# jai1215snu/ShiftedScaleQuantization

Hardware: AMD Instinct MI355X
Metric: Gelem/s shifted-scale q/dq + recon iters/s, ResNet-18 W2A4; top-1 vs ref (higher is better)
Workload: dtype f32; 1 GPU; resnet18 W2A4 bias_cal+bias_ch_quant, 1024 calib samples: A4 per-tensor q/dq of act [1024,64,56,56] + W2 per-channel q/dq of all 21 conv/fc weights (8-bit stem/head); parallelism=dp1

## Files before the change

shiftedscalequantization_amd/csrc/conv_wgrad.hip:

```cpp
#include <stdlib.h>

#include <algorithm>
#include <type_traits>

#include "ssq_common.h"

namespace ssq {

typedef float f32x16 __attribute__((ext_vector_type(16)));

constexpr int kUnr = 2;

struct WgradGeo {
  int Nb, C, H, W, Co, OH, OW, R, S, st, pad, G, Cig, Cog;
  int Ncol;
  int WM;
  int Pq;
  int lda;
  int chunks_per_n;
  int nchunks;
  int cps;
  int nsplit;
  int in_rows;
  int ci_span;
// ... 574 lines not shown
        const int rr = (int)fdiv((uint32_t)rem, dWp), cc = rem - rr * Wp;
        const int ih = rr - pad, iw = cc - pad;
        v[u] = 0.0f;
        if (e < tot && ih >= 0 && ih < H && iw >= 0 && iw < W) v[u] = xb[(int64_t)j * C * HW + ih * W + iw];
      }
#pragma unroll
      for (int u = 0; u < U; ++u)
        if (e0 + 256 * u < tot) xs[e0 + 256 * u] = v[u];
    }
    __syncthreads();
    for (int p0 = tid; p0 < totp; p0 += 256 * kPf) {
      float g[kPf];
#pragma unroll
      for (int k = 0; k < kPf; ++k) {
        const int p = p0 + 256 * k;
        const int j = (int)fdiv((uint32_t)p, dOHW);
        g[k] = 0.0f;
        if (p < totp) g[k] = db[(int64_t)j * C * OHW + (p - j * OHW)];
      }
#pragma unroll 1
      for (int k = 0; k < kPf; ++k) {
        const int p = p0 + 256 * k;
        if (p >= totp) break;
        const int j = (int)fdiv((uint32_t)p, dOHW), q = p - j * OHW;
        const int oh = (int)fdiv((uint32_t)q, dOW), ow = q - oh * OW;
        const float* xr = xs + j * HpWp + oh * st * Wp + ow * st;
#pragma unroll
        for (int kk = 0; kk < RSMAX; ++kk) {
          if (kk < RS) {
            const int r = kk / S, q2 = kk - r * S;
            acc[kk] = __fadd_rn(acc[kk], __fmul_rn(g[0], xr[r * Wp + q2]));
          }
        }
#pragma unroll
        for (int t = 0; t + 1 < kPf; ++t) g[t] = g[t + 1];
      }
    }
  }
#pragma unroll
  for (int j = 0; j < RSMAX; ++j) {
    float v = acc[j];
#pragma unroll
    for (int o = 32; o >= 1; o >>= 1) v = __fadd_rn(v, __shfl_xor(v, o));
    if (lane == 0) red[w][j] = v;
  }
  __syncthreads();
  if (tid < RS)
    part[((int64_t)split * C + c) * RS + tid] =
        __fadd_rn(__fadd_rn(__fadd_rn(red[0][tid], red[1][tid]), red[2][tid]), red[3][tid]);
}

static bool is_depthwise(int64_t C, int64_t Co, int64_t G) { return G == C && G == Co && G > 1; }
static int dw_stage(int64_t H, int64_t W, int64_t pad, int spl) {
  const int64_t b = (H + 2 * pad) * (W + 2 * pad) * (int64_t)sizeof(float);
  if (b > 4096) return 0;
  return (int)std::max<int64_t>(1, std::min<int64_t>(spl, 32 * 1024 / b));
}
static int dw_band_rows(int64_t H, int64_t W, int64_t R, int64_t st, int64_t pad, int64_t OH) {
  const int64_t Wp = W + 2 * pad, row = Wp * (int64_t)sizeof(float);
  if ((H + 2 * pad) * row <= 8192) return (int)OH;
  const int64_t rows = std::max<int64_t>(R, 8192 / row);
  return (int)std::min<int64_t>(OH, (rows - R) / st + 1);
}
static bool dw_lds_ok(int64_t H, int64_t W, int64_t pad) {
  return (H + 2 * pad) * (W + 2 * pad) * (int64_t)sizeof(float) <= 128 * 1024;
}

static int dw_splits(int64_t Nb, int64_t C, int* spl) {
  int64_t ns = std::max<int64_t>(1, std::min<int64_t>(Nb, (1024 + C - 1) / C));
  *spl = (int)((Nb + ns - 1) / ns);
  while (Nb % *spl) ++*spl;
  return (int)(Nb / *spl);
}

static size_t wgrad_lds(int wm, int pq, int64_t xtile) {
  return sizeof(float) * (2 * (size_t)(64 * wm) * (pq + 1) + 2 * (size_t)(xtile + 1));
}

static int wgrad_plan(int64_t Nb, int64_t C, int64_t H, int64_t W, int64_t Co, int64_t R,
                      int64_t S, int64_t st, int64_t pad, int64_t G, WgradGeo& g,
                      size_t* lds_bytes) {
  SSQ_REQUIRE(Nb >= 1 && C >= 1 && H >= 1 && W >= 1 && Co >= 1 && R >= 1 && S >= 1 && st >= 1 &&
                  pad >= 0 && G >= 1 && C % G == 0 && Co % G == 0,
              SSQ_E_ARG, "ssq_conv_wgrad: bad geometry");
  const int64_t OH = (H + 2 * pad - R) / st + 1, OW = (W + 2 * pad - S) / st + 1;
  SSQ_REQUIRE(OH >= 1 && OW >= 1 && Nb * C * H * W < (1ll << 31) && Nb * Co * OH * OW < (1ll << 31),
              SSQ_E_ARG, "ssq_conv_wgrad: sizes");
  g.Nb = (int)Nb; g.C = (int)C; g.H = (int)H; g.W = (int)W; g.Co = (int)Co;
  g.OH = (int)OH; g.OW = (int)OW; g.R = (int)R; g.S = (int)S; g.st = (int)st; g.pad = (int)pad;
  g.G = (int)G; g.Cig = (int)(C / G); g.Cog = (int)(Co / G);
  g.Ncol = g.Cig * g.R * g.S;
  const int RS = g.R * g.S;
  const int64_t Wp = W + 2 * pad;
  static const int64_t max_lds = [] {
    const char* v = getenv("SSQ_K17_MAXLDS");
    return (int64_t)(v && *v ? atoll(v) : 160 * 1024);
  }();
  double best = 1e300;
  for (int wm : {1, 2, 4}) {
    for (int pq : {128, 64}) {
      const int TM = 64 * wm, TN = 256 / wm;
      const int64_t span = std::min<int64_t>(g.Cig, (TN - 1) / RS + 2);
      const int64_t orows = (pq - 1 + OW - 1) / OW + 1;
      const int64_t in_rows = (orows - 1) * st + R;
      const int64_t xtile = span * in_rows * Wp;
      if ((int64_t)wgrad_lds(wm, pq, xtile) > max_lds) continue;
      const int64_t cpn = (OH * OW + pq - 1) / pq;
      const int64_t tiles = ((g.Cog + TM - 1) / TM) * ((g.Ncol + TN - 1) / TN);
      const double dma = (double)(std::min<int64_t>(TM, g.Cog) * ((pq + 63) / 64) +
                                  span * in_rows * ((W + 63) / 64)) / 4.0;
      const double cost = (double)tiles * Nb * (2.0 * OH * OW + cpn * (40.0 + dma));
      if (cost < best) {
        best = cost;
        g.WM = wm;
        g.Pq = pq;
        g.ci_span = (int)span;
        g.in_rows = (int)in_rows;
        g.xtile = (int)xtile;
      }
    }
  }
  SSQ_REQUIRE(best < 1e300, SSQ_E_ARG, "ssq_conv_wgrad: input rows too wide for the LDS tile");
  const int TM = 64 * g.WM, TN = 256 / g.WM;
  g.lda = g.Pq + 1;
  g.chunks_per_n = (int)((OH * OW + g.Pq - 1) / g.Pq);
  g.nchunks = g.Nb * g.chunks_per_n;
  g.m_tiles = (g.Cog + TM - 1) / TM;
  g.n_tiles = (g.Ncol + TN - 1) / TN;
  const int64_t tiles = (int64_t)g.n_tiles * g.m_tiles * g.G;
  int nsplit = (int)std::max<int64_t>(1, std::min<int64_t>(g.nchunks / 2, (512 + tiles - 1) / tiles));
  g.cps = (g.nchunks + nsplit - 1) / nsplit;
  g.nsplit = (g.nchunks + g.cps - 1) / g.cps;
  *lds_bytes = wgrad_lds(g.WM, g.Pq, g.xtile);
  return SSQ_OK;
}

constexpr int kBandMaxNI = 20;
__device__ float g_band_zero_page[4 * 64];

struct BandGeo {
  int C, H, W, Co, OW, OHW, Cig, Cog;
  int RB, Q, Qp, PA, IR, PXrow, PXci;
  int TMc, CBc;
  int bufsz;
  int d16;
  int ni_w;
  int bands_per_n, nchunks, cps, nsplit, m_tiles, n_tiles, remap;
  FastDiv dPA, dPXci, dPXrow;
};

template <int N>
using IntC = std::integral_constant<int, N>;

template <int WMX, int ST, int V, int NWV>
__global__ __launch_bounds__(64 * NWV, 1) void wgrad_band_stage1(const float* __restrict__ x,
                                                                 const float* __restrict__ dy,
                                                                 BandGeo g, float* __restrict__ part) {
  static_assert(NWV == 4 || NWV == 8, "4 or 8 waves");
  constexpr int WNX = 4 / WMX;
  constexpr int kSlots = kBandMaxNI * 4 / NWV;
  extern __shared__ float lds[];
  const int tid = threadIdx.x, lane = tid & 63;
  const int wave = __builtin_amdgcn_readfirstlane(tid >> 6);
  const int wt = wave & 3, role = wave >> 2;
  const int wm = wt / WNX, wn = wt - wm * WNX;
  int wg = blockIdx.x;
  const int tiles = g.m_tiles * g.n_tiles;
  if (g.remap) {
    const int per = (int)gridDim.x >> 3;
    wg = (wg & 7) * per + (wg >> 3);
  }
  const int split = wg / tiles, tile = wg - split * tiles;
  const int mt = tile / g.n_tiles, nt = tile - mt * g.n_tiles;
  const int co0 = mt * g.TMc, ci0 = nt * g.CBc;
  const int c_begin = split * g.cps, c_end = min(c_begin + g.cps, g.nchunks);
  const int abytes = g.TMc * g.PA;
  const int n16 = g.d16 ? min(kSlots, (g.bufsz / 256 - wave + NWV - 1) / NWV) : 0;
  const int n4 = g.d16 ? 0 : (g.bufsz / 64 - wave + NWV - 1) / NWV;

  int soff[kSlots], meta[kSlots];
#pragma unroll
  for (int i = 0; i < kSlots; ++i) {
    soff[i] = 0;
    meta[i] = 0;
    if (i < n16) {
      const int o = (wave + NWV * i) * 256 + lane * 4;
      if (o < abytes) {
        const int row = (int)fdiv((uint32_t)o, g.dPA), col = o - row * g.PA;
        if (col < g.Q && co0 + row < g.Cog) {
          soff[i] = (co0 + row) * g.OHW + col;
          meta[i] = 1;
        }
      } else {
        const int o2 = o - abytes;
        const int cl = (int)fdiv((uint32_t)o2, g.dPXci), rem = o2 - cl * g.PXci;
        const int ir = (int)fdiv((uint32_t)rem, g.dPXrow), iw = rem - ir * g.PXrow - 4;
        if (cl < g.CBc && ci0 + cl < g.Cig && ir < g.IR && iw >= 0 && iw < g.W) {
          soff[i] = ((ci0 + cl) * g.H + ir) * g.W + iw;
          meta[i] = 2 | (ir << 2);
        }
      }
    }
  }
  struct Band {
    const float* ab;
    const float* xb;
    int ih0;
  };
  auto band_of = [&](int c) {
    const int n = c / g.bands_per_n;
    const int oh0 = (c - n * g.bands_per_n) * g.RB;
    const int ih0 = oh0 * ST - 1;
    return Band{dy + (int64_t)n * g.Co * g.OHW + oh0 * g.OW,
                x + (int64_t)n * g.C * g.H * g.W + (int64_t)ih0 * g.W, ih0};
  };
  auto stage16 = [&](const Band& bd, int b) {
    const float* zero = g_band_zero_page + lane * 4;
    float* dst = lds + b * g.bufsz + wave * 256;
#pragma unroll
    for (int i = 0; i < kSlots; ++i) {
      if (i < n16) {
        const int kind = meta[i] & 3;
        const unsigned ih = (unsigned)(bd.ih0 + (meta[i] >> 2));
        const bool ok = (kind == 1) | ((kind == 2) & (ih < (unsigned)g.H));
        const uint64_t pa = (uint64_t)(bd.ab + soff[i]), px = (uint64_t)(bd.xb + soff[i]);
        const uint64_t p = ok ? (kind == 1 ? pa : px) : (uint64_t)zero;
        __builtin_amdgcn_global_load_lds((const void*)p, (void*)(dst + i * NWV * 256), 16, 0, 0);
      }
    }
  };
  const int HW = g.H * g.W;
  auto stage4 = [&](const Band& bd, int b, int i0, int i1) {
    const float* zero = g_band_zero_page + lane;
    float* dst = lds + b * g.bufsz + wave * 64;
    for (int i = i0; i < i1; ++i) {
      const int o = (wave + NWV * i) * 64 + lane;
      const float* src = zero;
      if ((wave + NWV * i) * 64 < abytes) {
        const int row = (int)fdiv((uint32_t)o, g.dPA), col = o - row * g.PA;
        if (col < g.Q && co0 + row < g.Cog) src = bd.ab + (co0 + row) * g.OHW + col;
      } else {
        const int o2 = o - abytes;
        const int cl = (int)fdiv((uint32_t)o2, g.dPXci), rem = o2 - cl * g.PXci;
        const int ir = (int)fdiv((uint32_t)rem, g.dPXrow), iw = rem - ir * g.PXrow - 4;
        const unsigned ih = (unsigned)(bd.ih0 + ir);
        if (cl < g.CBc && ci0 + cl < g.Cig && ir < g.IR && iw >= 0 && iw < g.W &&
            ih < (unsigned)g.H)
          src = bd.xb + (ci0 + cl) * HW + ir * g.W + iw;
      }
      __builtin_amdgcn_global_load_lds((const void*)src, (void*)(dst + i * NWV * 64), 4, 0, 0);
    }
  };

  typedef float f32x4v __attribute__((ext_vector_type(4)));
  typedef float f32x2v __attribute__((ext_vector_type(2)));
  const int h = lane >> 5, l32 = lane & 31;
  const int arow = (wm * 32 + l32) * g.PA;
  const int xrow = abytes + (wn * 32 + l32) * g.PXci;
  const int q0 = h * (g.Qp >> 1);
  const int ngroups = g.Qp / (2 * V);
  const int last_row = (g.Q - 1) / g.OW, last_col = (g.Q - 1) - last_row * g.OW;
  constexpr int NW = (V - 1) * ST + 3;
  const int per_step = (n4 + max(1, ngroups / 2) - 1) / max(1, ngroups / 2);
  if (c_begin < c_end) {
    const Band bd = band_of(c_begin);
    if (g.d16) stage16(bd, 0);
    else stage4(bd, 0, 0, n4);
  }

  auto body = [&](auto t0c, auto t1c) {
    constexpr int T0 = decltype(t0c)::value, T1 = decltype(t1c)::value, NT = T1 - T0;
    constexpr int R0 = T0 / 3, NR = (T1 - 1) / 3 - R0 + 1;
    f32x16 acc[NT];
#pragma unroll
    for (int t = 0; t < NT; ++t) acc[t] = f32x16{0};
    auto fetch = [&](const float* L, int q, int orow, int ow, float (&a)[V],
                     float (&w)[NR][NW]) {
      if constexpr (V == 4) {
        const f32x4v av = *(const f32x4v*)(L + arow + q);
        a[0] = av.x; a[1] = av.y; a[2] = av.z; a[3] = av.w;
      } else if constexpr (V == 2) {
        const f32x2v av = *(const f32x2v*)(L + arow + q);
        a[0] = av.x; a[1] = av.y;
      } else {
        a[0] = L[arow + q];
      }
      int xr_row = orow, xr_col = ow;
      if (q >= g.Q) {
        xr_row = last_row;
        xr_col = last_col - (V - 1);
      }
      const float* xr0 = L + xrow + (xr_row * ST + R0) * g.PXrow + xr_col * ST + 3;
#pragma unroll
      for (int r = 0; r < NR; ++r) {
        const float* xr = xr0 + r * g.PXrow;
        if constexpr (V == 4) {
          w[r][0] = xr[0];
          const f32x4v t1 = *(const f32x4v*)(xr + 1);
          w[r][1] = t1.x; w[r][2] = t1.y; w[r][3] = t1.z; w[r][4] = t1.w;
          if constexpr (ST == 1) {
            w[r][5] = xr[5];
          } else {
            const f32x4v t2 = *(const f32x4v*)(xr + 5);
            w[r][5] = t2.x; w[r][6] = t2.y; w[r][7] = t2.z; w[r][8] = t2.w;
          }
        } else {
#pragma unroll
          for (int j = 0; j < NW; ++j) w[r][j] = xr[j];
        }
      }
    };
    auto mfmas = [&](const float (&a)[V], const float (&w)[NR][NW]) {
#pragma unroll
      for (int r = 0; r < NR; ++r)
#pragma unroll
        for (int v = 0; v < V; ++v)
#pragma unroll
          for (int s = 0; s < 3; ++s) {
            const int tap = (R0 + r) * 3 + s;
            if (tap >= T0 && tap < T1)
              acc[tap - T0] = __builtin_amdgcn_mfma_f32_32x32x2f32(a[v], w[r][v * ST + s],
                                                                   acc[tap - T0], 0, 0, 0);
          }
    };
    auto interleave = [&]() {
      constexpr int NM = NT * V, ND = NM < 12 ? NM : 12;
#pragma unroll
      for (int k = 0; k < ND; ++k) {
        __builtin_amdgcn_sched_group_barrier(0x008, 1, 0);
        __builtin_amdgcn_sched_group_barrier(0x100, 1, 0);
      }
      __builtin_amdgcn_sched_group_barrier(0x008, NM - ND, 0);
    };
    for (int c = c_begin; c < c_end; ++c) {
      const int b = (c - c_begin) & 1;
      asm volatile("s_waitcnt vmcnt(0)" ::: "memory");
      __syncthreads();
      const bool more = c + 1 < c_end;
      const Band nb = band_of(more ? c + 1 : c);
      if (more && g.d16) stage16(nb, b ^ 1);
      const float* L = lds + b * g.bufsz;
      int q = q0, orow = q0 / g.OW, ow = q0 - orow * g.OW;
      auto advance = [&]() {
        q += V;
        ow += V;
        if (ow == g.OW) {
          ow = 0;
          ++orow;
        }
      };
      auto stage_slice = [&](int gi) {
        if (more && !g.d16) {
          const int i0 = gi * per_step;
          if (i0 < n4) stage4(nb, b ^ 1, i0, min(i0 + per_step, n4));
        }
      };
      float a0[V], w0[NR][NW], a1[V], w1[NR][NW];
      fetch(L, q, orow, ow, a0, w0);
      const int npairs = ngroups >> 1;
      for (int gp = 0; gp < npairs; ++gp) {
        stage_slice(2 * gp);
        advance();
        fetch(L, q, orow, ow, a1, w1);
        mfmas(a0, w0);
        interleave();
        stage_slice(2 * gp + 1);
        advance();
        fetch(L, q, orow, ow, a0, w0);
        mfmas(a1, w1);
        interleave();
      }
      if (ngroups & 1) {
        stage_slice(ngroups - 1);
        mfmas(a0, w0);
      }
    }
    const int co_w = co0 + wm * 32, ci = ci0 + wn * 32 + l32;
    if (ci < g.Cig) {
#pragma unroll
      for (int t = 0; t < NT; ++t) {
        float* dst = part + ((int64_t)split * 9 + T0 + t) * g.Cog * g.Cig;
#pragma unroll
        for (int i = 0; i < 16; ++i) {
          const int co = co_w + (i & 3) + 8 * (i >> 2) + 4 * h;
          if (co < g.Cog) dst[(int64_t)co * g.Cig + ci] = acc[t][i];
        }
      }
    }
  };
  if constexpr (NWV == 4) {
    body(IntC<0>{}, IntC<9>{});
  } else {
    if (role == 0) body(IntC<0>{}, IntC<5>{});
    else body(IntC<5>{}, IntC<9>{});
  }
}

static int g_wgrad_form = 0;
static int band_waves() {
  static const int w = [] {
    const char* e = getenv("SSQ_BAND_WAVES");
    return e && *e && atoi(e) == 4 ? 4 : 8;
  }();
  return g_wgrad_form == 4 ? 4 : w;
}

static int band_plan(int64_t Nb, int64_t C, int64_t H, int64_t W, int64_t Co, int64_t R,
                     int64_t S, int64_t st, int64_t pad, int64_t G, BandGeo& g, int* wmx,
                     int* vpx) {
  if (G != 1 || R != 3 || S != 3 || pad != 1 || (st != 1 && st != 2)) return 0;
  const int64_t OH = (H + 2 - 3) / st + 1, OW = (W + 2 - 3) / st + 1;
  if (OH < 1 || OW < 1 || Co % 32 || C % 32) return 0;
  if (Nb * C * H * W >= (1ll << 31) || Nb * Co * OH * OW >= (1ll << 31)) return 0;
  g.C = (int)C; g.H = (int)H; g.W = (int)W; g.Co = (int)Co; g.OW = (int)OW;
  g.OHW = (int)(OH * OW); g.Cig = (int)C; g.Cog = (int)Co;
  const int V = OW % 4 == 0 ? 4 : (OW % 2 == 0 ? 2 : 1);
  auto odd4 = [](int v) { v = (v + 3) / 4 * 4; return (v / 4) % 2 ? v : v + 4; };
  const int64_t budget = 160 * 1024 / 2 / 4;
  bool found = false;
  double best = 1e300;
  for (int wm : {2, 4}) {
    const int TMc = 32 * wm, CBc = 32 * (4 / wm);
    if (wm == 4 && Co < 128) continue;
    for (int rb = (int)std::min<int64_t>(OH, 8); rb >= 1; --rb) {
      if (OH % rb) continue;
      const int Q = rb * (int)OW, Qp = (Q + 2 * V - 1) / (2 * V) * (2 * V);
      const int IR = (rb - 1) * (int)st + 3;
      const bool d16 = W % 4 == 0 && g.OHW % 4 == 0 && Q % 4 == 0 && Qp == Q;
      const int need = (int)((OW - 1) * st) + 6;
      const int PXrow = d16 ? (int)W + 8 : (std::max<int>(need, (int)W + 4) + 3) / 4 * 4;
      const int PA = odd4(Qp + 1), PXci = odd4(IR * PXrow);
      const int64_t buf = ((int64_t)TMc * PA + (int64_t)CBc * PXci + 1023) / 1024 * 1024;
      if (buf > budget) continue;
      const int ni = d16 ? (int)(buf / 1024) : (int)(buf / 256);
      if (d16 && ni > kBandMaxNI) continue;
      const double cost = (288.0 * Qp + 1500.0 + (d16 ? 40.0 : 10.0) * ni) / Q;
      if (cost >= best) continue;
      best = cost;
      g.RB = rb; g.Q = Q; g.Qp = Qp; g.PA = PA; g.IR = IR; g.PXrow = PXrow; g.PXci = PXci;
      g.TMc = TMc; g.CBc = CBc; g.bufsz = (int)buf; g.d16 = d16 ? 1 : 0; g.ni_w = ni;
      *wmx = wm;
      *vpx = V;
      found = true;
    }
  }
  if (!found) return 0;
  g.dPA = make_fastdiv((uint32_t)g.PA);
  g.dPXci = make_fastdiv((uint32_t)g.PXci);
  g.dPXrow = make_fastdiv((uint32_t)g.PXrow);
  g.m_tiles = (g.Cog + g.TMc - 1) / g.TMc;
  g.n_tiles = (g.Cig + g.CBc - 1) / g.CBc;
  g.bands_per_n = (int)(OH / g.RB);
  g.nchunks = (int)Nb * g.bands_per_n;
  const int tiles = g.m_tiles * g.n_tiles;
  int ns = std::max(1, std::min(g.nchunks, (256 + tiles - 1) / tiles));
  g.cps = (g.nchunks + ns - 1) / ns;
  g.nsplit = (g.nchunks + g.cps - 1) / g.cps;
  g.remap = ((int64_t)g.nsplit * tiles) % 8 == 0;
  return 1;
}

static bool use_band(int64_t Nb, int64_t C, int64_t H, int64_t W, int64_t Co, int64_t R,
                     int64_t S, int64_t st, int64_t pad, int64_t G, BandGeo& g, int* wmx,
                     int* vpx) {
  if (g_wgrad_form != 0 && g_wgrad_form != 3 && g_wgrad_form != 4) return false;
  return band_plan(Nb, C, H, W, Co, R, S, st, pad, G, g, wmx, vpx) != 0;
}
static bool use_i2c(int64_t R, int64_t S, int64_t Co, int64_t G) {
  if (g_wgrad_form != 0) return g_wgrad_form == 2;
  return R * S > 1 && G == 1 && Co >= 128;
}

}

using namespace ssq;

extern "C" int ssq_conv_wgrad_set_form(int form) {
  const int old = g_wgrad_form;
  if (form >= 0 && form <= 4) g_wgrad_form = form;
  return old;
}

extern "C" int ssq_conv_wgrad_kind(int64_t Nb, int64_t C, int64_t H, int64_t W, int64_t Co,
                                   int64_t R, int64_t S, int64_t stride, int64_t pad,
                                   int64_t groups) {
  if (is_depthwise(C, Co, groups) && R * S <= 25 && Nb >= 1 && dw_lds_ok(H, W, pad)) return 5;
  BandGeo gb;
  int wmx, vpx;
  if (use_band(Nb, C, H, W, Co, R, S, stride, pad, groups, gb, &wmx, &vpx)) return gb.d16 ? 3 : 6;
  if (use_i2c(R, S, Co, groups)) {
    I2cGeo gi;
    return wgrad_i2c_plan(Nb, C, H, W, Co, R, S, stride, pad, groups, gi) ? 0 : 2;
  }
  if (R == 1 && S == 1 && pad == 0) {
    W1Geo g1;
    return wgrad_1x1_plan(Nb, C, H, W, Co, stride, groups, g1) ? 0 : 4;
  }
  WgradGeo g;
  size_t lds;
  return wgrad_plan(Nb, C, H, W, Co, R, S, stride, pad, groups, g, &lds) ? 0 : 1;
}

extern "C" size_t ssq_conv_wgrad_workspace_size(int64_t Nb, int64_t C, int64_t H, int64_t W,
                                                int64_t Co, int64_t R, int64_t S, int64_t stride,
                                                int64_t pad, int64_t groups) {
  if (is_depthwise(C, Co, groups) && R * S <= 25 && Nb >= 1 && dw_lds_ok(H, W, pad)) {
    int spl;
    const int ns = dw_splits(Nb, C, &spl);
    const int64_t OH = (H + 2 * pad - R) / stride + 1;
    int64_t nbands = 1;
    if (dw_stage(H, W, pad, spl) == 0 && OH >= 1) {
      const int bh = dw_band_rows(H, W, R, stride, pad, OH);
      nbands = (OH + bh - 1) / bh;
    }
    return (size_t)ns * (size_t)nbands * (size_t)C * (size_t)(R * S) * sizeof(float);
  }
  {
    BandGeo gb;
    int wmx, vpx;
    if (use_band(Nb, C, H, W, Co, R, S, stride, pad, groups, gb, &wmx, &vpx))
      return (size_t)gb.nsplit * 9 * (size_t)Co * (size_t)C * sizeof(float);
  }
  if (use_i2c(R, S, Co, groups)) {
    I2cGeo gi;
    int wm;
    if (wgrad_i2c_plan(Nb, C, H, W, Co, R, S, stride, pad, groups, gi)) return 0;
    wgrad_i2c_tiles(gi, &wm);
    return (size_t)gi.nsplit * (size_t)Co * (size_t)gi.Ncol * sizeof(float);
  }
  if (R == 1 && S == 1 && pad == 0) {
    W1Geo g1;
    if (wgrad_1x1_plan(Nb, C, H, W, Co, stride, groups, g1)) return 0;
    return (size_t)g1.nsplit * (size_t)Co * (size_t)g1.Cig * sizeof(float);
  }
  WgradGeo g;
  size_t lds;
  if (wgrad_plan(Nb, C, H, W, Co, R, S, stride, pad, groups, g, &lds)) return 0;
  return (size_t)g.nsplit * (size_t)Co * (size_t)g.Ncol * sizeof(float);
}

extern "C" int ssq_conv_wgrad(const float* x, const float* dy, int64_t Nb, int64_t C, int64_t H,
                              int64_t W, int64_t Co, int64_t R, int64_t S, int64_t stride,
                              int64_t pad, int64_t groups, float* dw, void* ws, size_t ws_bytes,
                              ssq_stream_t stream) {
  SSQ_REQUIRE(x && dy && dw, SSQ_E_ARG, "ssq_conv_wgrad: null pointer");
  hipStream_t s = (hipStream_t)stream;
  if (is_depthwise(C, Co, groups) && R * S <= 25 && dw_lds_ok(H, W, pad)) {
    SSQ_REQUIRE(Nb >= 1 && H >= 1 && W >= 1 && stride >= 1 && pad >= 0, SSQ_E_ARG,
                "ssq_conv_wgrad: bad geometry");
    const int64_t OH = (H + 2 * pad - R) / stride + 1, OW = (W + 2 * pad - S) / stride + 1;
    SSQ_REQUIRE(OH >= 1 && OW >= 1 && Nb * C * H * W < (1ll << 31) && Nb * C * OH * OW < (1ll << 31),
                SSQ_E_ARG, "ssq_conv_wgrad: sizes");
    int spl;
    const int ns = dw_splits(Nb, C, &spl);
    const size_t need = (size_t)ns * (size_t)C * (size_t)(R * S) * sizeof(float);
    SSQ_REQUIRE(ws && ws_bytes >= need, SSQ_E_WS, "ssq_conv_wgrad: workspace too small");
    const dim3 grid((unsigned)C, (unsigned)ns);
    const int64_t plane = (H + 2 * pad) * (W + 2 * pad);
    const int nb = dw_stage(H, W, pad, spl);
    if (nb > 0) {
      const size_t lds = (size_t)nb * plane * sizeof(float);
      const FastDiv dWp = make_fastdiv((uint32_t)(W + 2 * pad)), dP = make_fastdiv((uint32_t)plane),
                    dOHW = make_fastdiv((uint32_t)(OH * OW)), dOW = make_fastdiv((uint32_t)OW);
      if (R * S <= 9)
        hipLaunchKernelGGL(wgrad_dw_small<9>, grid, dim3(256), lds, s, x, dy, (int)C, (int)H,
                           (int)W, (int)OH, (int)OW, (int)R, (int)S, (int)stride, (int)pad, spl,
                           nb, dWp, dP, dOHW, dOW, (float*)ws);
      else
        hipLaunchKernelGGL(wgrad_dw_small<25>, grid, dim3(256), lds, s, x, dy, (int)C, (int)H,
                           (int)W, (int)OH, (int)OW, (int)R, (int)S, (int)stride, (int)pad, spl,
                           nb, dWp, dP, dOHW, dOW, (float*)ws);
      const int64_t n = C * R * S;
      hipLaunchKernelGGL(wgrad_stage2, dim3((unsigned)std::min<int64_t>((n + 63) / 64, 4096)),
                         dim3(256), 0, s, (const float*)ws, ns, n, dw);
      return check_launch("ssq_conv_wgrad");
    }
    const int bh = dw_band_rows(H, W, R, stride, pad, OH);
    const int nbands = (int)((OH + bh - 1) / bh);
    SSQ_REQUIRE(ws_bytes >= need * (size_t)nbands, SSQ_E_WS, "ssq_conv_wgrad: workspace too small");
    const dim3 gridb((unsigned)C, (unsigned)(ns * nbands));
    const size_t lds = (size_t)(((int64_t)bh - 1) * stride + R) * (W + 2 * pad) * sizeof(float);
    static bool dw_attr = false;
    if (!dw_attr) {
      hipFuncSetAttribute((const void*)wgrad_dw_stage1<9>,
                          hipFuncAttributeMaxDynamicSharedMemorySize, 128 * 1024);
      hipFuncSetAttribute((const void*)wgrad_dw_stage1<25>,
                          hipFuncAttributeMaxDynamicSharedMemorySize, 128 * 1024);
      dw_attr = true;
    }
    if (R * S <= 9)
      hipLaunchKernelGGL(wgrad_dw_stage1<9>, gridb, dim3(256), lds, s, x, dy, (int)C, (int)H, (int)W,
                         (int)OH, (int)OW, (int)R, (int)S, (int)stride, (int)pad, spl, bh, nbands,
                         make_fastdiv((uint32_t)(W + 2 * pad)), (float*)ws);
    else
      hipLaunchKernelGGL(wgrad_dw_stage1<25>, gridb, dim3(256), lds, s, x, dy, (int)C, (int)H, (int)W,
                         (int)OH, (int)OW, (int)R, (int)S, (int)stride, (int)pad, spl, bh, nbands,
                         make_fastdiv((uint32_t)(W + 2 * pad)), (float*)ws);
    const int64_t n = C * R * S;
    hipLaunchKernelGGL(wgrad_stage2, dim3((unsigned)std::min<int64_t>((n + 63) / 64, 4096)),
                       dim3(256), 0, s, (const float*)ws, ns * nbands, n, dw);
    return check_launch("ssq_conv_wgrad");
  }
  {
    BandGeo gb;
    int wmx, vpx;
    if (use_band(Nb, C, H, W, Co, R, S, stride, pad, groups, gb, &wmx, &vpx)) {
      const size_t needb = (size_t)gb.nsplit * 9 * (size_t)Co * (size_t)C * sizeof(float);
      SSQ_REQUIRE(ws && ws_bytes >= needb, SSQ_E_WS, "ssq_conv_wgrad: workspace too small");
      typedef void (*BandK)(const float*, const float*, BandGeo, float*);
#define SSQ_BK(NWV)                                                                          \
  {{{wgrad_band_stage1<2, 1, 4, NWV>, wgrad_band_stage1<2, 1, 2, NWV>,                        \
     wgrad_band_stage1<2, 1, 1, NWV>},                                                        \
    {wgrad_band_stage1<2, 2, 4, NWV>, wgrad_band_stage1<2, 2, 2, NWV>,                        \
     wgrad_band_stage1<2, 2, 1, NWV>}},                                                       \
   {{wgrad_band_stage1<4, 1, 4, NWV>, wgrad_band_stage1<4, 1, 2, NWV>,                        \
     wgrad_band_stage1<4, 1, 1, NWV>},                                                        \
    {wgrad_band_stage1<4, 2, 4, NWV>, wgrad_band_stage1<4, 2, 2, NWV>,                        \
     wgrad_band_stage1<4, 2, 1, NWV>}}}
      static const BandK kernels[2][2][2][3] = {SSQ_BK(4), SSQ_BK(8)};
#undef SSQ_BK
      static bool band_attr = false;
      if (!band_attr) {
        for (auto& a0 : kernels)
          for (auto& a : a0)
            for (auto& b : a)
              for (BandK k : b)
                hipFuncSetAttribute((const void*)k, hipFuncAttributeMaxDynamicSharedMemorySize,
                                    160 * 1024);
        band_attr = true;
      }
      const int w8 = band_waves() == 8;
      const BandK kb = kernels[w8][wmx == 4][stride == 2][vpx == 4 ? 0 : (vpx == 2 ? 1 : 2)];
      const dim3 gridb((unsigned)(gb.nsplit * gb.m_tiles * gb.n_tiles));
      const size_t ldsb = 2 * (size_t)gb.bufsz * sizeof(float);
      hipLaunchKernelGGL(kb, gridb, dim3(w8 ? 512 : 256), ldsb, s, x, dy, gb, (float*)ws);
      const int64_t inner = Co * C, nb = 9 * inner;
      hipLaunchKernelGGL(wgrad_stage2, dim3((unsigned)std::min<int64_t>((nb + 63) / 64, 4096)),
                         dim3(256), 0, s, (const float*)ws, gb.nsplit, nb, dw, inner, 9);
      return check_launch("ssq_conv_wgrad");
    }
  }
  if (use_i2c(R, S, Co, groups)) {
    I2cGeo gi;
    int wm;
    const int rci = wgrad_i2c_plan(Nb, C, H, W, Co, R, S, stride, pad, groups, gi);
    if (rci) return rci;
    wgrad_i2c_tiles(gi, &wm);
    const size_t needi = (size_t)gi.nsplit * (size_t)Co * (size_t)gi.Ncol * sizeof(float);
    SSQ_REQUIRE(ws && ws_bytes >= needi, SSQ_E_WS, "ssq_conv_wgrad: workspace too small");
    const dim3 gridi(gi.n_tiles, gi.m_tiles * gi.G, gi.nsplit);
    (void)wm;
    hipLaunchKernelGGL(wgrad_i2c_stage1<2>, gridi, dim3(256), 0, s, x, dy, gi, (float*)ws);
    const int64_t ni = (int64_t)Co * gi.Ncol;
    hipLaunchKernelGGL(wgrad_stage2, dim3((unsigned)std::min<int64_t>((ni + 63) / 64, 4096)),
                       dim3(256), 0, s, (const float*)ws, gi.nsplit, ni, dw);
    return check_launch("ssq_conv_wgrad");
  }
  if (R == 1 && S == 1 && pad == 0) {
    W1Geo g1;
    const int rc1 = wgrad_1x1_plan(Nb, C, H, W, Co, stride, groups, g1);
    if (rc1) return rc1;
    const size_t need1 = (size_t)g1.nsplit * (size_t)Co * (size_t)g1.Cig * sizeof(float);
    SSQ_REQUIRE(ws && ws_bytes >= need1, SSQ_E_WS, "ssq_conv_wgrad: workspace too small");
    const dim3 grid1(g1.n_tiles, g1.m_tiles * g1.G, g1.nsplit);
    hipLaunchKernelGGL(wgrad_1x1_stage1<2>, grid1, dim3(256), 0, s, x, dy, g1, (float*)ws);
    const int64_t n1 = (int64_t)Co * g1.Cig;
    hipLaunchKernelGGL(wgrad_stage2, dim3((unsigned)std::min<int64_t>((n1 + 63) / 64, 4096)),
                       dim3(256), 0, s, (const float*)ws, g1.nsplit, n1, dw);
    return check_launch("ssq_conv_wgrad");
  }
  WgradGeo g;
  size_t lds;
  int rc = wgrad_plan(Nb, C, H, W, Co, R, S, stride, pad, groups, g, &lds);
  if (rc) return rc;
  const size_t need = (size_t)g.nsplit * (size_t)Co * (size_t)g.Ncol * sizeof(float);
  SSQ_REQUIRE(ws && ws_bytes >= need, SSQ_E_WS, "ssq_conv_wgrad: workspace too small");
  static bool lds_attr = false;
  if (!lds_attr) {
    hipFuncSetAttribute((const void*)wgrad_stage1<1>, hipFuncAttributeMaxDynamicSharedMemorySize,
                        160 * 1024);
    hipFuncSetAttribute((const void*)wgrad_stage1<2>, hipFuncAttributeMaxDynamicSharedMemorySize,
                        160 * 1024);
    hipFuncSetAttribute((const void*)wgrad_stage1<4>, hipFuncAttributeMaxDynamicSharedMemorySize,
                        160 * 1024);
    lds_attr = true;
  }
  const dim3 grid(g.n_tiles, g.m_tiles * g.G, g.nsplit);
  if (g.WM == 1)
    hipLaunchKernelGGL(wgrad_stage1<1>, grid, dim3(256), lds, s, x, dy, g, (float*)ws);
  else if (g.WM == 2)
    hipLaunchKernelGGL(wgrad_stage1<2>, grid, dim3(256), lds, s, x, dy, g, (float*)ws);
  else
    hipLaunchKernelGGL(wgrad_stage1<4>, grid, dim3(256), lds, s, x, dy, g, (float*)ws);
  const int64_t n = (int64_t)Co * g.Ncol;
  hipLaunchKernelGGL(wgrad_stage2, dim3((unsigned)std::min<int64_t>((n + 63) / 64, 4096)),
                     dim3(256), 0, s, (const float*)ws, g.nsplit, n, dw);
  return check_launch("ssq_conv_wgrad");
}

__global__ __launch_bounds__(kBlock) void wgrad_gemm_operands(
    const float* __restrict__ x, const float* __restrict__ dy, uint32_t C, uint32_t H,
    uint32_t W, uint32_t Co, uint32_t R, uint32_t S, uint32_t st, int pad, uint32_t OW,
    uint32_t NP, FastDiv dRS, FastDiv dS, FastDiv dP, FastDiv dOW, uint32_t CRS,
    uint32_t P, uint32_t nb1, uint32_t tiles_k, uint32_t vec4, float* __restrict__ col,
    float* __restrict__ dy2) {
  if (blockIdx.x < nb1) {
    __shared__ float tile[64][65];
    const uint32_t tk = blockIdx.x % tiles_k, tp = blockIdx.x / tiles_k;
    const uint32_t row0 = tp * 64, k0 = tk * 64, RS = R * S;
    const uint32_t pp = threadIdx.x & 63, kb = threadIdx.x >> 6, row = row0 + pp;
    const bool rok = row < NP;
    const uint32_t n = rok ? fdiv(row, dP) : 0u, p = row - n * P;
    const uint32_t oh = fdiv(p, dOW), ow = p - oh * OW;
    const int ih0 = (int)(oh * st) - pad, iw0 = (int)(ow * st) - pad;
    const float* xn = x + (size_t)n * C * H * W;
    float v[16];
#pragma unroll
    for (int j = 0; j < 16; ++j) {
      const uint32_t k = k0 + kb + 4 * j;
      const uint32_t ci = fdiv(k, dRS), rs = k - ci * RS;
      const uint32_t r = fdiv(rs, dS), sc = rs - r * S;
      const int ih = ih0 + (int)r, iw = iw0 + (int)sc;
      v[j] = 0.0f;
      if (rok && k < CRS && ih >= 0 && ih < (int)H && iw >= 0 && iw < (int)W)
        v[j] = xn[((size_t)ci * H + ih) * W + iw];
    }
#pragma unroll
    for (int j = 0; j < 16; ++j) tile[kb + 4 * j][pp] = v[j];
    __syncthreads();
    if (vec4) {
      for (uint32_t i = threadIdx.x; i < 64 * 16; i += kBlock) {
        const uint32_t pp = i >> 4, kq = (i & 15) << 2;
        const uint32_t row = row0 + pp, k = k0 + kq;
        if (row < NP && k < CRS)
          *reinterpret_cast<float4*>(col + (size_t)row * CRS + k) =
              make_float4(tile[kq][pp], tile[kq + 1][pp], tile[kq + 2][pp], tile[kq + 3][pp]);
      }
    } else {
      for (uint32_t i = threadIdx.x; i < 64 * 64; i += kBlock) {
        const uint32_t pp = i >> 6, kk = i & 63;
        const uint32_t row = row0 + pp, k = k0 + kk;
        if (row < NP && k < CRS) col[(size_t)row * CRS + k] = tile[kk][pp];
      }
    }
    return;
  }
  const uint32_t nb2 = gridDim.x - nb1;
  const uint32_t n2 = Co * NP;
  for (uint32_t e = (blockIdx.x - nb1) * kBlock + threadIdx.x; e < n2; e += nb2 * kBlock) {
    const uint32_t co = e / NP, q = e - co * NP;
    const uint32_t n = fdiv(q, dP), p = q - n * P;
    dy2[e] = dy[((size_t)n * Co + co) * P + p];
  }
}

template <int ACT>
__device__ __forceinline__ float epi_in(float v, uint32_t c, const float* __restrict__ bias,
                                        const float* __restrict__ gamma,
                                        const float* __restrict__ phi, bool quant,
                                        const QParams& qp) {
  float t = bias ? __fadd_rn(v, bias[c]) : v;
  if (gamma) t = __fadd_rn(__fmul_rn(t, gamma[c]), phi[c]);
  t = act_fwd<ACT>(t);
  if (quant) {
    float q;
    t = fq1(t, qp, &q);
  }
  return t;
}

template <int ACT>
__global__ __launch_bounds__(kBlock) void gemm_col_epi(
    const float* __restrict__ y, const float* __restrict__ bias, const float* __restrict__ gamma,
    const float* __restrict__ phi, const float* __restrict__ qdelta,
    const float* __restrict__ qzp, float qlo, float qhi, uint32_t C, uint32_t H, uint32_t W,
    uint32_t R, uint32_t S, uint32_t st, int pad, uint32_t OW, uint32_t NP, FastDiv dCRS,
    FastDiv dRS, FastDiv dS, FastDiv dP, FastDiv dOW, uint32_t CRS, uint32_t P,
    float* __restrict__ col) {
  const bool quant = qdelta != nullptr;
  QParams qp{1.0f, 0.0f, qlo, qhi};
  if (quant) {
    qp.d = qdelta[0];
    qp.z = qzp[0];
  }
  const uint32_t n1 = NP * CRS;
// ... 73 lines not shown
```

shiftedscalequantization_amd/kernels.py:

```python
import collections
import ctypes as C
import functools
import os

import torch

from . import _capi as A
from ._capi import call, fptr, query, stream_of, workspace
from .nets import GlobalMeanPool


def qrange(n_bits, sym):
    n = 2 ** n_bits
    return (-(n // 2), n // 2 - 1) if sym else (0, n - 1)


def geometry(w):
    if w.dim() == 4:
        return int(w.shape[0]), int(w.shape[1]), int(w.shape[2] * w.shape[3]), 0
    if w.dim() == 2:
        return int(w.shape[0]), int(w.shape[1]), 1, 1
    raise ValueError(f"weight must be 2-D (Linear) or 4-D (Conv2d), got {tuple(w.shape)}")


# ... 2151 lines not shown


WGRAD_GEMM = "auto"


def _use_wgrad_gemm(x, weight, stride, padding, groups=1, geo=None):
    g = geo or conv_geometry(x.shape, weight.shape, stride, padding, 1, groups)
    if WGRAD_GEMM != "auto" or WGRAD_POLICY == "never" or groups != 1 or not g.single:
        return False
    NP, crs = g.Nb * g.OH * g.OW, g.Cig * g.R * g.S
    if NP * crs >= (1 << 31) or g.Co * NP >= (1 << 31) or g.OH * g.OW > 196:
        return False
    if g.R * g.S == 1:
        return g.Co >= 256 or (g.OH * g.OW <= 49 and torch.backends.cudnn.deterministic)
    return g.Co >= 128 and crs >= 1152


def _use_wgrad_bmm(x, weight, stride, padding, groups=1, geo=None):
    g = geo or conv_geometry(x.shape, weight.shape, stride, padding, 1, groups)
    if WGRAD_POLICY != "auto" or groups != 1 or (g.R, g.S, g.st, g.pad) != (1, 1, 1, 0):
        return False
    p = g.H * g.W
    return p >= 400 or (p >= 100 and torch.backends.cudnn.deterministic)


def _use_dgrad_1x1(x, weight, stride, padding, groups=1, geo=None):
    g = geo or conv_geometry(x.shape, weight.shape, stride, padding, 1, groups)
    if WGRAD_POLICY == "never" or groups != 1 or not torch.backends.cudnn.deterministic:
        return False
    if (g.R, g.S, g.st, g.pad) != (1, 1, 1, 0) or not _dev_f32(x):
        return False
    co, c, p = g.Co, g.Cig, g.H * g.W
    if p >= 12544:
        return True
    if p <= 49:
        return co <= 4 * c
    if 196 <= p <= 784:
        return c >= 128 and co >= c and (p >= 784 or co >= 2 * c)
    return False


def conv1x1_dgrad_gemm(dy, weight):
    n, co, h, w = (int(v) for v in dy.shape)
    c = int(weight.shape[1])
    gx = torch.matmul(weight.detach().reshape(co, c).t(), dy.reshape(n, co, h * w))
    return gx.view(n, c, h, w)


def conv_wgrad_1x1_bmm(x, dy, w_shape):
    n, c = int(x.shape[0]), int(x.shape[1])
    co, p = int(w_shape[0]), int(x.shape[2] * x.shape[3])
    gw = torch.matmul(dy.detach().reshape(n, co, p), x.detach().reshape(n, c, p).transpose(1, 2))
    return gw.sum(0).view(tuple(w_shape))


def _use_wgrad_grouped_gemm(x, weight, stride, padding, groups=1, geo=None):
    g = geo or conv_geometry(x.shape, weight.shape, stride, padding, 1, groups)
    if WGRAD_POLICY != "auto" or groups <= 1 or g.Cig <= 1:
        return False
    NP = g.Nb * g.OH * g.OW
    if NP * g.Cig * groups * g.R * g.S >= (1 << 31) or g.Co * NP >= (1 << 31):
        return False
    return g.OH * g.OW <= 196


def conv_wgrad_grouped_gemm(x, dy, w_shape, stride, padding, groups, col=None):
    Co, Cig, R, S = (int(v) for v in w_shape)
    c2, dy2 = gemm_operands(x, dy, (Co, Cig * groups, R, S), stride, padding,
                            want_col=col is None, want_dy2=True)
    col = c2 if col is None else col
    NP = col.shape[0]
    a = dy2.view(groups, Co // groups, NP)
    b = col.view(NP, groups, Cig * R * S).transpose(0, 1)
    return torch.matmul(a, b).reshape(tuple(w_shape))


def conv_fwd_grouped_gemm(x, weight, stride, padding, groups):
    g = conv_geometry(x.shape, weight.shape, stride, padding, 1, groups)
    k = g.Cig * g.R * g.S
    col, _ = gemm_operands(x, None, (g.Co, g.Cig * groups, g.R, g.S), stride, padding,
                           want_col=True, want_dy2=False)
    y = torch.matmul(weight.detach().reshape(groups, g.Co // groups, k),
                     col.view(-1, groups, k).permute(1, 2, 0))
    y = y.view(groups, g.Co // groups, g.Nb, g.OH * g.OW).permute(2, 0, 1, 3).contiguous()
    return y.view(g.Nb, g.Co, g.OH, g.OW), col


def _use_fwd_gemm(x, weight, stride, padding, groups=1):
    return (weight.shape[2] * weight.shape[3] > 1
            and _use_wgrad_gemm(x, weight, stride, padding, groups))


FWD_1X1_GEMM = os.environ.get("SSQ_FWD_1X1_GEMM", "1") != "0"


def _use_fwd_1x1(x, weight, stride, padding, dilation, groups, geo=None):
    g = geo or conv_geometry(x.shape, weight.shape, stride, padding, dilation, groups)
    if not FWD_1X1_GEMM or WGRAD_POLICY == "never" or groups != 1 or not _dev_f32(x):
        return False
    if (g.R, g.S, g.pad, g.dil) != (1, 1, 0, 1) or g.st < 2:
        return False
    return not (100 < g.OH * g.OW < 400 and g.Nb < 128)


def conv1x1_fwd_gemm(x, weight, stride, keep_xs=False):
    st = conv_geometry(x.shape, weight.shape, stride, 0).st
    xs = x[:, :, ::st, ::st].contiguous()
    n, c, oh, ow = xs.shape
    co = int(weight.shape[0])
    y = torch.matmul(weight.detach().reshape(co, c), xs.view(n, c, oh * ow))
    y = y.view(n, co, oh, ow)
    return (y, xs) if keep_xs else y


def _use_wgrad_bmm_s2(x, weight, stride, padding, groups=1, geo=None):
    g = geo or conv_geometry(x.shape, weight.shape, stride, padding, 1, groups)
    if WGRAD_POLICY != "auto" or groups != 1 or (g.R, g.S, g.pad) != (1, 1, 0) or g.st < 2:
        return False
    return g.OH * g.OW >= 400 and g.Cig % 64 == 0 and g.Co % 64 == 0


ConvRoute = collections.namedtuple("ConvRoute", "geo fwd dx dw")


def conv_route(x, weight, stride, padding, dilation, groups, need_dx, need_dw):
    g = conv_geometry(x.shape, weight.shape, stride, padding, dilation, groups)
    a = (x, weight, stride, padding)
    ours = need_dw and g.dil == 1
    gemm = ours and _use_wgrad_gemm(*a, groups, g)
    if getattr(x, "_ssq_epi", None) is not None and gemm and g.R * g.S > 1:
        return ConvRoute(g, "epi_gemm", "lib" if need_dx else None, "im2col_gemm")
    if groups > 1 and dwconv_supported(*a, dilation, groups, g) and x.is_contiguous():
        return ConvRoute(g, "k18", "k18" if need_dx else None, "k17" if need_dw else None)
    if ours:
        grouped = not gemm and _use_wgrad_grouped_gemm(*a, groups, g)
        if gemm or grouped or (conv_wgrad_supported(*a, dilation, groups, g) and _k17_rule(g)):
            fwd = "im2col_gemm" if gemm and g.R * g.S > 1 else "grouped_gemm" if grouped else \
                "gemm_1x1" if _use_fwd_1x1(*a, dilation, groups, g) else "lib"
            dw = "im2col_gemm" if gemm else "bmm_1x1" if _use_wgrad_bmm(*a, groups, g) else \
                "bmm_s2" if fwd == "gemm_1x1" and _use_wgrad_bmm_s2(*a, groups, g) else \
                "grouped_gemm" if grouped else "k17"
            dx = None if not need_dx else "gemm_1x1" if _use_dgrad_1x1(*a, groups, g) else "lib"
            return ConvRoute(g, fwd, dx, dw)
    if need_dx and _use_dgrad_1x1(*a, groups, g):
        return ConvRoute(g, "lib", "gemm_1x1", "lib" if need_dw else None)
    fwd = "gemm_1x1" if not (need_dx or need_dw) and _use_fwd_1x1(*a, dilation, groups, g) \
        else "lib"
    return ConvRoute(g, fwd, "lib" if need_dx else None, "lib" if need_dw else None)


def _k17_rule(g):
    if WGRAD_POLICY != "auto":
        return WGRAD_POLICY == "always"
    if g.groups > 1 or wgrad_kind(g[:4], g[4:8], g.st, g.pad, g.groups, g) == 3:
        return True
    return torch.backends.cudnn.deterministic and (g.st > 1 or g.OH * g.OW >= 100)


def conv2d(x, weight, stride=1, padding=0, dilation=1, groups=1):
    grad, lazy = torch.is_grad_enabled(), getattr(x, "_ssq_epi", None) is not None
    route = conv_route(x, weight, stride, padding, dilation, groups,
                       grad and (lazy or x.requires_grad), grad and weight.requires_grad)
    if route.fwd == "epi_gemm":
        return epi_conv_gemm(x, weight, stride, padding)
    if lazy:
        x = materialize_epi(x)
    if route.fwd == "k18":
        if route.dx or route.dw:
            return DwConv2dFn.apply(x, weight, stride, padding)
        return dwconv_fwd(x, weight, stride, padding)
    if route.dw not in (None, "lib") or route.dx == "gemm_1x1":
        return Conv2dFn.apply(x, weight, stride, padding, dilation, groups, route)
    if route.fwd == "gemm_1x1":
        return conv1x1_fwd_gemm(x, weight, stride)
    return torch.nn.functional.conv2d(x, weight, None, stride, padding, dilation, groups)
```

Before: 700.4 Gelem/s.

## Add split-bf16 MFMA path for band wgrad kernel on stride-1 wide layers

Adds a band wgrad variant that splits each fp32 operand into three bf16 parts (high, mid, low) and accumulates six bf16 32x32x16 MFMAs per tap. This gives near-fp32 accuracy while using the higher-throughput bf16 matrix instructions instead of the fp32 MFMA path. It runs by default for stride-1 layers with OW >= 28 when 16-byte staging applies. In exchange it adds conversion ALU work and extra register pressure, and rounding differs slightly from true fp32.

```diff
diff --git a/shiftedscalequantization_amd/csrc/conv_wgrad.hip b/shiftedscalequantization_amd/csrc/conv_wgrad.hip
--- a/shiftedscalequantization_amd/csrc/conv_wgrad.hip
+++ b/shiftedscalequantization_amd/csrc/conv_wgrad.hip
@@ -750,11 +750,48 @@
 template <int N>
 using IntC = std::integral_constant<int, N>;
 
-template <int WMX, int ST, int V, int NWV>
+typedef __bf16 bf16x8 __attribute__((ext_vector_type(8)));
+typedef uint32_t u32x4 __attribute__((ext_vector_type(4)));
+
+__device__ __forceinline__ uint32_t cvt_pk_bf16(float lo, float hi) {
+  typedef __bf16 bf16x2 __attribute__((ext_vector_type(2)));
+  typedef float f32x2v __attribute__((ext_vector_type(2)));
+  return __builtin_bit_cast(uint32_t, __builtin_convertvector(f32x2v{lo, hi}, bf16x2));
+}
+
+__device__ __forceinline__ float sub_f32(float a, float b) {
+  float r;
+  asm("v_sub_f32 %0, %1, %2" : "=v"(r) : "v"(a), "v"(b));
+  return r;
+}
+
+template <int N>
+__device__ __forceinline__ void split_levels(float (&lv)[3][N]) {
+#pragma unroll
+  for (int k = 0; k < 2; ++k)
+#pragma unroll
+    for (int i = 0; i < N; i += 2) {
+      const int j = i + 1 < N ? i + 1 : i;
+      const uint32_t p = cvt_pk_bf16(lv[k][i], lv[k][j]);
+      lv[k + 1][i] = sub_f32(lv[k][i], __uint_as_float(p << 16));
+      if (j != i) lv[k + 1][j] = sub_f32(lv[k][j], __uint_as_float(p & 0xffff0000u));
+    }
+}
+
+template <int D, int N>
+__device__ __forceinline__ bf16x8 pack8(const float (&lv)[N], int i0) {
+  u32x4 p;
+#pragma unroll
+  for (int j = 0; j < 4; ++j) p[j] = cvt_pk_bf16(lv[i0 + D * 2 * j], lv[i0 + D * (2 * j + 1)]);
+  return __builtin_bit_cast(bf16x8, p);
+}
+
+template <int WMX, int ST, int V, int NWV, bool SPLIT = false>
 __global__ __launch_bounds__(64 * NWV, 1) void wgrad_band_stage1(const float* __restrict__ x,
                                                                  const float* __restrict__ dy,
                                                                  BandGeo g, float* __restrict__ part) {
   static_assert(NWV == 4 || NWV == 8, "4 or 8 waves");
+  static_assert(!SPLIT || (NWV == 8 && V == 4), "the split form: 8 waves, 16-B staging");
   constexpr int WNX = 4 / WMX;
   constexpr int kSlots = kBandMaxNI * 4 / NWV;
   extern __shared__ float lds[];
@@ -865,6 +902,119 @@
     if (g.d16) stage16(bd, 0);
     else stage4(bd, 0, 0, n4);
   }
+
+  auto store_part = [&](auto t0c, const auto& acc) {
+    constexpr int T0 = decltype(t0c)::value;
+    constexpr int NT = (int)(sizeof(acc) / sizeof(acc[0]));
+    const int co_w = co0 + wm * 32, ci = ci0 + wn * 32 + l32;
+    if (ci < g.Cig) {
+#pragma unroll
+      for (int t = 0; t < NT; ++t) {
+        float* dst = part + ((int64_t)split * 9 + T0 + t) * g.Cog * g.Cig;
+#pragma unroll
+        for (int i = 0; i < 16; ++i) {
+          const int co = co_w + (i & 3) + 8 * (i >> 2) + 4 * h;
+          if (co < g.Cog) dst[(int64_t)co * g.Cig + ci] = acc[t][i];
+        }
+      }
+    }
+  };
+
+  auto body_split = [&](auto t0c, auto t1c) {
+    constexpr int T0 = decltype(t0c)::value, T1 = decltype(t1c)::value, NT = T1 - T0;
+    constexpr int R0 = T0 / 3, NR = (T1 - 1) / 3 - R0 + 1;
+    constexpr int NWS = 7 * ST + 3;
+    f32x16 acc[NT];
+#pragma unroll
+    for (int t = 0; t < NT; ++t) acc[t] = f32x16{0};
+    const int G8 = (g.OW + 7) >> 3, NG = g.RB * G8, NGh = (NG + 1) >> 1;
+    auto fetch = [&](const float* L, int gi, int row, int k, float (&a)[8],
+                     float (&w)[NR][NWS]) {
+      const bool pad = gi >= NG;
+      if (pad) {
+        row = g.RB - 1;
+        k = G8 - 1;
+      }
+      const int col = min(8 * k, g.OW - 8);
+      const int j0 = pad ? 8 : 8 * k - col;
+      const float* ap = L + arow + row * g.OW + col;
+      const f32x4v lo = *(const f32x4v*)ap, hi = *(const f32x4v*)(ap + 4);
+#pragma unroll
+      for (int j = 0; j < 4; ++j) {
+        a[j] = j0 >= 4 ? 0.f : lo[j];
+        a[4 + j] = j0 >= 8 ? 0.f : hi[j];
+      }
+      const float* xr0 = L + xrow + (row * ST + R0) * g.PXrow + col * ST + 3;
+#pragma unroll
+      for (int r = 0; r < NR; ++r) {
+        const float* xr = xr0 + r * g.PXrow;
+        w[r][0] = xr[0];
+#pragma unroll
+        for (int b = 0; b < (NWS - 1) / 4; ++b) {
+          const f32x4v t = *(const f32x4v*)(xr + 1 + 4 * b);
+          w[r][1 + 4 * b] = t.x; w[r][2 + 4 * b] = t.y; w[r][3 + 4 * b] = t.z; w[r][4 + 4 * b] = t.w;
+        }
+        if constexpr (ST == 1) w[r][9] = xr[9];
+      }
+    };
+    auto compute = [&](const float (&a)[8], const float (&w)[NR][NWS]) {
+      float al[3][8];
+#pragma unroll
+      for (int j = 0; j < 8; ++j) al[0][j] = a[j];
+      split_levels(al);
+      const bf16x8 ah = pack8<1>(al[0], 0), am = pack8<1>(al[1], 0), a_l = pack8<1>(al[2], 0);
+#pragma unroll
+      for (int r = 0; r < NR; ++r) {
+        float wl[3][NWS];
+#pragma unroll
+        for (int j = 0; j < NWS; ++j) wl[0][j] = w[r][j];
+        split_levels(wl);
+#pragma unroll
+        for (int s = 0; s < 3; ++s) {
+          const int tap = (R0 + r) * 3 + s;
+          if (tap >= T0 && tap < T1) {
+            const bf16x8 bh = pack8<ST>(wl[0], s), bm = pack8<ST>(wl[1], s),
+                         bl = pack8<ST>(wl[2], s);
+            f32x16 c = acc[tap - T0];
+            c = __builtin_amdgcn_mfma_f32_32x32x16_bf16(am, bm, c, 0, 0, 0);
+            c = __builtin_amdgcn_mfma_f32_32x32x16_bf16(a_l, bh, c, 0, 0, 0);
+            c = __builtin_amdgcn_mfma_f32_32x32x16_bf16(ah, bl, c, 0, 0, 0);
+            c = __builtin_amdgcn_mfma_f32_32x32x16_bf16(am, bh, c, 0, 0, 0);
+            c = __builtin_amdgcn_mfma_f32_32x32x16_bf16(ah, bm, c, 0, 0, 0);
+            c = __builtin_amdgcn_mfma_f32_32x32x16_bf16(ah, bh, c, 0, 0, 0);
+            acc[tap - T0] = c;
+          }
+        }
+      }
+    };
+    for (int c = c_begin; c < c_end; ++c) {
+      const int b = (c - c_begin) & 1;
+      asm volatile("s_waitcnt vmcnt(0)" ::: "memory");
+      __syncthreads();
+      if (c + 1 < c_end) stage16(band_of(c + 1), b ^ 1);
+      const float* L = lds + b * g.bufsz;
+      int gi = h * NGh, row = gi / G8, k = gi - row * G8;
+      auto advance = [&]() {
+        ++gi;
+        if (++k == G8) {
+          k = 0;
+          ++row;
+        }
+      };
+      float a0[8], w0[NR][NWS], a1[8], w1[NR][NWS];
+      fetch(L, gi, row, k, a0, w0);
+      for (int gp = 0; gp < (NGh >> 1); ++gp) {
+        advance();
+        fetch(L, gi, row, k, a1, w1);
+        compute(a0, w0);
+        advance();
+        fetch(L, gi, row, k, a0, w0);
+        compute(a1, w1);
+      }
+      if (NGh & 1) compute(a0, w0);
+    }
+    store_part(t0c, acc);
+  };
 
   auto body = [&](auto t0c, auto t1c) {
     constexpr int T0 = decltype(t0c)::value, T1 = decltype(t1c)::value, NT = T1 - T0;
@@ -973,20 +1123,12 @@
         mfmas(a0, w0);
       }
     }
-    const int co_w = co0 + wm * 32, ci = ci0 + wn * 32 + l32;
-    if (ci < g.Cig) {
-#pragma unroll
-      for (int t = 0; t < NT; ++t) {
-        float* dst = part + ((int64_t)split * 9 + T0 + t) * g.Cog * g.Cig;
-#pragma unroll
-        for (int i = 0; i < 16; ++i) {
-          const int co = co_w + (i & 3) + 8 * (i >> 2) + 4 * h;
-          if (co < g.Cog) dst[(int64_t)co * g.Cig + ci] = acc[t][i];
-        }
-      }
-    }
+    store_part(t0c, acc);
   };
-  if constexpr (NWV == 4) {
+  if constexpr (SPLIT) {
+    if (role == 0) body_split(IntC<0>{}, IntC<5>{});
+    else body_split(IntC<5>{}, IntC<9>{});
+  } else if constexpr (NWV == 4) {
     body(IntC<0>{}, IntC<9>{});
   } else {
     if (role == 0) body(IntC<0>{}, IntC<5>{});
@@ -1061,8 +1203,17 @@
 static bool use_band(int64_t Nb, int64_t C, int64_t H, int64_t W, int64_t Co, int64_t R,
                      int64_t S, int64_t st, int64_t pad, int64_t G, BandGeo& g, int* wmx,
                      int* vpx) {
-  if (g_wgrad_form != 0 && g_wgrad_form != 3 && g_wgrad_form != 4) return false;
+  if (g_wgrad_form != 0 && g_wgrad_form < 3) return false;
   return band_plan(Nb, C, H, W, Co, R, S, st, pad, G, g, wmx, vpx) != 0;
+}
+static bool use_split(const BandGeo& g, int vpx, int64_t stride) {
+  if (!g.d16 || vpx != 4 || g.OW < 8) return false;
+  if (g_wgrad_form != 0) return g_wgrad_form == 5;
+  static const int knob = [] {
+    const char* e = getenv("SSQ_BAND_SPLIT");
+    return e && *e ? (atoi(e) != 0 ? 1 : 0) : -1;
+  }();
+  return knob >= 0 ? knob == 1 : (stride == 1 && g.OW >= 28);
 }
 static bool use_i2c(int64_t R, int64_t S, int64_t Co, int64_t G) {
   if (g_wgrad_form != 0) return g_wgrad_form == 2;
@@ -1075,7 +1226,7 @@
 
 extern "C" int ssq_conv_wgrad_set_form(int form) {
   const int old = g_wgrad_form;
-  if (form >= 0 && form <= 4) g_wgrad_form = form;
+  if (form >= 0 && form <= 5) g_wgrad_form = form;
   return old;
 }
 
@@ -1085,7 +1236,8 @@
   if (is_depthwise(C, Co, groups) && R * S <= 25 && Nb >= 1 && dw_lds_ok(H, W, pad)) return 5;
   BandGeo gb;
   int wmx, vpx;
-  if (use_band(Nb, C, H, W, Co, R, S, stride, pad, groups, gb, &wmx, &vpx)) return gb.d16 ? 3 : 6;
+  if (use_band(Nb, C, H, W, Co, R, S, stride, pad, groups, gb, &wmx, &vpx))
+    return use_split(gb, vpx, stride) ? 7 : (gb.d16 ? 3 : 6);
   if (use_i2c(R, S, Co, groups)) {
     I2cGeo gi;
     return wgrad_i2c_plan(Nb, C, H, W, Co, R, S, stride, pad, groups, gi) ? 0 : 2;
@@ -1227,8 +1379,21 @@
                                     160 * 1024);
         band_attr = true;
       }
-      const int w8 = band_waves() == 8;
-      const BandK kb = kernels[w8][wmx == 4][stride == 2][vpx == 4 ? 0 : (vpx == 2 ? 1 : 2)];
+      static const BandK split_kernels[2][2] = {
+          {wgrad_band_stage1<2, 1, 4, 8, true>, wgrad_band_stage1<2, 2, 4, 8, true>},
+          {wgrad_band_stage1<4, 1, 4, 8, true>, wgrad_band_stage1<4, 2, 4, 8, true>}};
+      static bool split_attr = false;
+      if (!split_attr) {
+        for (auto& a : split_kernels)
+          for (BandK k : a)
+            hipFuncSetAttribute((const void*)k, hipFuncAttributeMaxDynamicSharedMemorySize,
+                                160 * 1024);
+        split_attr = true;
+      }
+      const bool split = use_split(gb, vpx, stride);
+      const int w8 = split || band_waves() == 8;
+      const BandK kb = split ? split_kernels[wmx == 4][stride == 2]
+                             : kernels[w8][wmx == 4][stride == 2][vpx == 4 ? 0 : (vpx == 2 ? 1 : 2)];
       const dim3 gridb((unsigned)(gb.nsplit * gb.m_tiles * gb.n_tiles));
       const size_t ldsb = 2 * (size_t)gb.bufsz * sizeof(float);
       hipLaunchKernelGGL(kb, gridb, dim3(w8 ? 512 : 256), ldsb, s, x, dy, gb, (float*)ws);
diff --git a/shiftedscalequantization_amd/kernels.py b/shiftedscalequantization_amd/kernels.py
--- a/shiftedscalequantization_amd/kernels.py
+++ b/shiftedscalequantization_amd/kernels.py
@@ -2327,7 +2327,7 @@
 def _k17_rule(g):
     if WGRAD_POLICY != "auto":
         return WGRAD_POLICY == "always"
-    if g.groups > 1 or wgrad_kind(g[:4], g[4:8], g.st, g.pad, g.groups, g) == 3:
+    if g.groups > 1 or wgrad_kind(g[:4], g[4:8], g.st, g.pad, g.groups, g) in (3, 7):
         return True
     return torch.backends.cudnn.deterministic and (g.st > 1 or g.OH * g.OW >= 100)
 
```

Result: slower. 687.8 Gelem/s (-1.8%).
